# OpenDriveLab/ViDAR

Hardware: AMD Instinct MI355X
Metric: train samples/sec (6-cam->BEV step) (higher is better)
Workload: dtype f32

## Files before the change

### vidar_amd/csrc/dcn.hip

```cpp
#include <hip/hip_runtime.h>
#include <stdint.h>

#include "vidar_hip.h"
#include "vidar_common.h"
#include "det_scatter.h"

namespace {

struct PlaneTile { int plane, tile; bool ok; };
__device__ __forceinline__ PlaneTile xcd_plane_tile(int L, int T, int planes) {
  const int xcd = L & 7, j = L >> 3;
  const int pl = (j / T) * 8 + xcd;
  return PlaneTile{pl, j - (j / T) * T, pl < planes};
}
inline unsigned xcd_plane_grid(int T, int planes) { return 8u * (unsigned)T * (unsigned)((planes + 7) / 8); }

struct Conv { int C, H, W, Ho, Wo, kh, kw, stride, pad, dil; };

struct Bil {
  int h0, w0;
  float lh, lw;
  bool in, t, b, l, r;
};

__device__ __forceinline__ Bil bil(float h, float w, int H, int W) {
  Bil q;
  q.in = h > -1.f && w > -1.f && h < H && w < W;
  q.h0 = (int)floorf(h); q.w0 = (int)floorf(w);
  q.lh = h - q.h0; q.lw = w - q.w0;
  q.t = q.h0 >= 0; q.b = q.h0 + 1 <= H - 1; q.l = q.w0 >= 0; q.r = q.w0 + 1 <= W - 1;
  return q;
}

struct Pos { float h, w; };
__device__ __forceinline__ Pos tap_pos(const Conv& g, int py, int px, int t, float oh, float ow) {
  const int i = t / g.kw, j = t - i * g.kw;
  return Pos{py * g.stride - g.pad + i * g.dil + oh, px * g.stride - g.pad + j * g.dil + ow};
}

template <class F>
__device__ __forceinline__ void for_corners(const Bil& q, int W, F f) {
  const float hh = 1.f - q.lh, hw = 1.f - q.lw;
  const int tl = q.h0 * W + q.w0;
  if (q.t && q.l) f(tl, hh * hw);
  if (q.t && q.r) f(tl + 1, hh * q.lw);
  if (q.b && q.l) f(tl + W, q.lh * hw);
  if (q.b && q.r) f(tl + W + 1, q.lh * q.lw);
}

constexpr int kMaxTaps = 9;

typedef float pair_t __attribute__((ext_vector_type(2), aligned(4)));

template <bool PAIR>
__device__ __forceinline__ pair_t load_pair(const void* p) {
  if constexpr (PAIR) return *reinterpret_cast<const pair_t*>(p);
  else return pair_t{*reinterpret_cast<const float*>(p), 0.f};
}

struct PairMap {
  int top, bot;
  bool same, left;
  __device__ __forceinline__ float e0(float cl, float cr) const { return same ? cl : (left ? cr : 0.f); }
  __device__ __forceinline__ float e1(float cl, float cr) const { return same ? cr : (left ? 0.f : cl); }
};

__device__ __forceinline__ PairMap pair_map(const Bil& q, int H, int W) {
  const int c0 = min(max(q.w0, 0), max(W - 2, 0));
  const int r0 = min(max(q.h0, 0), H - 1), r1 = min(max(q.h0 + 1, 0), H - 1);
  return PairMap{r0 * W + c0, r1 * W + c0, q.w0 == c0, q.w0 < c0};
}

constexpr int kCP = 16;
struct TapFoot { unsigned top, bot; float wt0, wt1, wb0, wb1; };

__device__ __forceinline__ TapFoot tap_foot(Pos s, float m, const Conv& g) {
  const Bil q = bil(s.h, s.w, g.H, g.W);
  const PairMap pm = pair_map(q, g.H, g.W);
  const float wl = (q.l ? 1.f - q.lw : 0.f), wr = (q.r ? q.lw : 0.f);
  const float a0 = pm.e0(wl, wr), a1 = pm.e1(wl, wr);
  const float ht = (q.t ? 1.f - q.lh : 0.f) * m, hb = (q.b ? q.lh : 0.f) * m;
  TapFoot f;
  f.top = (unsigned)pm.top * 4u; f.bot = (unsigned)pm.bot * 4u;
  f.wt0 = q.in ? ht * a0 : 0.f; f.wt1 = q.in ? ht * a1 : 0.f;
  f.wb0 = q.in ? hb * a0 : 0.f; f.wb1 = q.in ? hb * a1 : 0.f;
  return f;
}

template <bool PAIR>
__device__ __forceinline__ void im2col_body(const float* __restrict__ x, const float* __restrict__ offset,
                                            const float* __restrict__ mask, float* __restrict__ cols, const Conv& g, int nimg) {
  const int P = g.Ho * g.Wo, K = g.kh * g.kw;
  const int cgroups = (g.C + kCP - 1) / kCP;
  const PlaneTile pt = xcd_plane_tile(blockIdx.x, (P + 255) / 256, cgroups * nimg);
  if (!pt.ok) return;
  const int p = pt.tile * 256 + threadIdx.x;
  if (p >= P) return;
  const int n = pt.plane / cgroups, c0 = (pt.plane - n * cgroups) * kCP, nc = min(kCP, g.C - c0);
  const int py = p / g.Wo, px = p % g.Wo;
  const size_t plane = (size_t)g.H * g.W, KP = (size_t)K * P;
  const char* im = reinterpret_cast<const char*>(x + ((size_t)n * g.C + c0) * plane);
  float* out = cols + ((size_t)n * g.C + c0) * KP + p;
  const float* off_n = offset + (size_t)n * 2 * K * P + p;
  const float* msk_n = mask + (size_t)n * K * P + p;
  float oh = off_n[0], ow = off_n[P], m = msk_n[0];
  for (int t = 0; t < K; ++t) {
    const TapFoot f = tap_foot(tap_pos(g, py, px, t, oh, ow), m, g);
    pair_t a[kCP], b[kCP];
#pragma unroll
    for (int c = 0; c < kCP; ++c) {
      const char* pl = im + (size_t)(c < nc ? c : 0) * plane * 4;
      a[c] = load_pair<PAIR>(pl + f.top);
      b[c] = load_pair<PAIR>(pl + f.bot);
    }
    if (t + 1 < K) {
      oh = off_n[(size_t)(2 * t + 2) * P]; ow = off_n[(size_t)(2 * t + 3) * P]; m = msk_n[(size_t)(t + 1) * P];
    }
#pragma unroll
    for (int c = 0; c < kCP; ++c)
      if (c < nc) {
        const float v = f.wt0 * a[c].x + f.wt1 * a[c].y + f.wb0 * b[c].x + f.wb1 * b[c].y;
        __builtin_nontemporal_store(v, out + (size_t)c * KP + (size_t)t * P);
      }
  }
}

__global__ __launch_bounds__(256) void dcn_im2col_pair_kernel(
    const float* __restrict__ x, const float* __restrict__ offset, const float* __restrict__ mask,
    float* __restrict__ cols, Conv g, int nimg) {
  im2col_body<true>(x, offset, mask, cols, g, nimg);
}
__global__ __launch_bounds__(256) void dcn_im2col_kernel(
    const float* __restrict__ x, const float* __restrict__ offset, const float* __restrict__ mask,
    float* __restrict__ cols, Conv g, int nimg) {
  im2col_body<false>(x, offset, mask, cols, g, nimg);
}

constexpr int kCG = 8;
template <class Acc>
__global__ __launch_bounds__(256) void dcn_col2im_kernel(const float* __restrict__ grad_cols, const float* __restrict__ offset,
                                                         const float* __restrict__ mask, float* __restrict__ grad_x, Conv g,
                                                         typename Acc::Param param) {
  Acc acc(grad_x, param);
  const int P = g.Ho * g.Wo, K = g.kh * g.kw;
  const int p = blockIdx.x * 256 + threadIdx.x;
  if constexpr (!Acc::kMeasureOnly) {
    if (p >= P) return;
  }
  const int n = blockIdx.z, c0 = blockIdx.y * kCG, nc = min(kCG, g.C - c0);
  const int py = p / g.Wo, px = p % g.Wo;
  const size_t plane = (size_t)g.H * g.W, KP = (size_t)K * P;
  float* gim = grad_x + ((size_t)n * g.C + c0) * plane;
  const float* gc = grad_cols + ((size_t)n * g.C + c0) * KP + p;
  for (int t = 0; t < K; ++t) {
    if constexpr (Acc::kMeasureOnly) {
      if (p >= P) break;
    }
    const size_t o = ((size_t)n * 2 * K + 2 * t) * P + p;
    const Pos s = tap_pos(g, py, px, t, offset[o], offset[o + P]);
    const Bil q = bil(s.h, s.w, g.H, g.W);
    if (!q.in) continue;
    const float m = mask[((size_t)n * K + t) * P + p];
    for (int c = 0; c < nc; ++c) {
      const float gv = gc[(size_t)c * KP + (size_t)t * P] * m;
      if (gv == 0.f) continue;
      for_corners(q, g.W, [&](int pix, float w) { acc.add(gim + (size_t)c * plane + pix, w * gv); });
    }
  }
  acc.flush();
}

struct Entry { int src; float w; };

template <bool FILL>
__global__ __launch_bounds__(256) void dcn_revmap_kernel(const float* __restrict__ offset,
                                                         const float* __restrict__ mask, int* __restrict__ cursor,
                                                         Entry* __restrict__ rec, Conv g) {
  const int P = g.Ho * g.Wo, K = g.kh * g.kw, HW = g.H * g.W;
  const int p = blockIdx.x * 256 + threadIdx.x;
  if (p >= P) return;
  const int t = blockIdx.y, n = blockIdx.z;
  const int py = p / g.Wo, px = p % g.Wo;
  const size_t o = ((size_t)n * 2 * K + 2 * t) * P + p;
  const Pos s = tap_pos(g, py, px, t, offset[o], offset[o + P]);
  const Bil q = bil(s.h, s.w, g.H, g.W);
  if (!q.in) return;
  const float m = FILL ? mask[((size_t)n * K + t) * P + p] : 0.f;
  int* cur = cursor + ((size_t)n * K + t) * HW;
  const int src = t * P + p;
  for_corners(q, g.W, [&](int pix, float w) {
    if (FILL) rec[atomicAdd(cur + pix, 1)] = Entry{src, w * m};
    else atomicAdd(cur + pix, 1);
  });
}

__global__ __launch_bounds__(1024) void dcn_revmap_scan_kernel(int* __restrict__ cursor, int* __restrict__ first,
                                                               int HW, int per_image) {
  __shared__ int s_part[1024];
  const int n = blockIdx.x;
  int* cnt = cursor + (size_t)n * HW;
  int* fst = first + (size_t)n * HW;
  const int per = (HW + 1023) / 1024;
  const int r0 = min(HW, (int)threadIdx.x * per), r1 = min(HW, r0 + per);
  int sum = 0;
  for (int i = r0; i < r1; ++i) sum += cnt[i];
  s_part[threadIdx.x] = sum;
  __syncthreads();
  for (int d = 1; d < 1024; d <<= 1) {
    const int a = (int)threadIdx.x >= d ? s_part[threadIdx.x - d] : 0;
    __syncthreads();
    s_part[threadIdx.x] += a;
    __syncthreads();
  }
  int run = n * per_image + s_part[threadIdx.x] - sum;
  for (int i = r0; i < r1; ++i) { const int c = cnt[i]; fst[i] = run; cnt[i] = run; run += c; }
}

constexpr int kGC = 16;
__global__ __launch_bounds__(256) void dcn_col2im_gather_kernel(const float* __restrict__ grad_cols,
                                                                const int* __restrict__ first,
                                                                const int* __restrict__ last,
                                                                const Entry* __restrict__ rec,
                                                                float* __restrict__ grad_x, Conv g) {
  const int P = g.Ho * g.Wo, K = g.kh * g.kw, HW = g.H * g.W;
  const int pix = blockIdx.x * 256 + threadIdx.x;
  if (pix >= HW) return;
  const int n = blockIdx.z, c0 = blockIdx.y * kGC;
  float acc[kGC];
#pragma unroll
  for (int c = 0; c < kGC; ++c) acc[c] = 0.f;
  const size_t KP = (size_t)K * P;
  const float* gc = grad_cols + ((size_t)n * g.C + c0) * KP;
  const int nc = min(kGC, g.C - c0);
  for (int t = 0; t < K; ++t) {
    const size_t bin = ((size_t)n * K + t) * HW + pix;
    const int e0 = first[bin], e1 = last[bin];
    if (nc == kGC) {
      int e = e0;
      for (; e + 1 < e1; e += 2) {
        const Entry r0 = rec[e], r1 = rec[e + 1];
        float v0[kGC], v1[kGC];
#pragma unroll
        for (int c = 0; c < kGC; ++c) { v0[c] = gc[(size_t)c * KP + r0.src]; v1[c] = gc[(size_t)c * KP + r1.src]; }
#pragma unroll
        for (int c = 0; c < kGC; ++c) acc[c] += r0.w * v0[c] + r1.w * v1[c];
      }
      if (e < e1) {
        const Entry r = rec[e];
#pragma unroll
        for (int c = 0; c < kGC; ++c) acc[c] += r.w * gc[(size_t)c * KP + r.src];
      }
    } else {
      for (int e = e0; e < e1; ++e) {
        const Entry r = rec[e];
        for (int c = 0; c < nc; ++c) acc[c] += r.w * gc[(size_t)c * KP + r.src];
      }
    }
  }
  for (int c = 0; c < nc; ++c) grad_x[((size_t)n * g.C + c0 + c) * HW + pix] = acc[c];
}

#ifndef VIDAR_DCN_GRY
#define VIDAR_DCN_GRY 2
#endif
#ifndef VIDAR_DCN_GLC
#define VIDAR_DCN_GLC 8
#endif
constexpr int kGRY = VIDAR_DCN_GRY;
constexpr int kGTH = 8 * kGRY, kGTW = 32;
#ifndef VIDAR_DCN_GHALO
#define VIDAR_DCN_GHALO 5
#endif
constexpr int kGHalo = VIDAR_DCN_GHALO;
constexpr int kGWH = kGTH + 2 * kGHalo + 2;
constexpr int kGWW = kGTW + 2 * kGHalo + 2;
constexpr int kGWP = (kGWW + 3) / 4 * 4;
constexpr int kGWS = kGWH * kGWP;
constexpr int kGLC = VIDAR_DCN_GLC;
constexpr int kGPos = (kGWS + 255) / 256;

__global__ __launch_bounds__(256) void dcn_col2im_gather_lds_kernel(
    const float* __restrict__ grad_cols, const int* __restrict__ first, const int* __restrict__ last,
    const Entry* __restrict__ rec, float* __restrict__ grad_x, Conv g, int tiles_x, int tiles_y, int nimg, float inv_wo) {
  __shared__ __attribute__((aligned(16))) float s_gc[kGLC * kGWS];
  constexpr int K = 9;
  const int P = g.Ho * g.Wo, HW = g.H * g.W;
  const int cgroups = (g.C + kGLC - 1) / kGLC;
  const PlaneTile pt = xcd_plane_tile(blockIdx.x, tiles_x * tiles_y, cgroups * nimg);
  if (!pt.ok) return;
  const int tile = pt.tile, tyi = tile / tiles_x, txi = tile - tyi * tiles_x;
  const int n = pt.plane / cgroups, c0 = (pt.plane - n * cgroups) * kGLC, nc = min(kGLC, g.C - c0);
  const int ry = threadIdx.x / kGTW, rx = threadIdx.x % kGTW;
  const int dx = txi * kGTW + rx;
  const size_t KP = (size_t)K * P;
  const float* gc = grad_cols + ((size_t)n * g.C + c0) * KP;
  float acc[kGRY][kGLC];
#pragma unroll
  for (int k = 0; k < kGRY; ++k)
#pragma unroll
    for (int c = 0; c < kGLC; ++c) acc[k][c] = 0.f;
  for (int t = 0; t < K; ++t) {
    const int i = t / 3, j = t - i * 3;
    const int wy0 = tyi * kGTH + g.pad - i - kGHalo - 1, wx0 = txi * kGTW + g.pad - j - kGHalo - 1;
    const float* gct = gc + (size_t)t * P;
    __syncthreads();
    {
      const int wave = __builtin_amdgcn_readfirstlane((int)threadIdx.x >> 6);
#pragma unroll
      for (int k = 0; k < kGPos; ++k) {
        const int e = threadIdx.x + k * 256;
        const int r = e / kGWP, cc = e - r * kGWP;
        const int sy = wy0 + r, sx = wx0 + cc;
        const bool ok = e < kGWS && sy >= 0 && sy < g.Ho && sx >= 0 && sx < g.Wo && cc < kGWW;
        const int off = ok ? sy * g.Wo + sx : 0;
        if (ok) {
#pragma unroll
          for (int c = 0; c < kGLC; ++c)
            __builtin_amdgcn_global_load_lds((const __attribute__((address_space(1))) void*)(gct + (size_t)(c < nc ? c : 0) * KP + off),
                                             (__attribute__((address_space(3))) void*)(s_gc + c * kGWS + k * 256 + wave * 64), 4, 0, 0);
        }
      }
    }
    __syncthreads();
    if (dx >= g.W) continue;
#pragma unroll
    for (int k = 0; k < kGRY; ++k) {
      const int dy = tyi * kGTH + ry + 8 * k;
      if (dy >= g.H) continue;
      const size_t bin = ((size_t)n * K + t) * HW + dy * g.W + dx;
      const int e1 = last[bin];
      int e = first[bin];
      Entry nxt = e < e1 ? rec[e] : Entry{0, 0.f};
      while (e < e1) {
        const Entry r = nxt;
        ++e;
        if (e < e1) nxt = rec[e];
        const int p = r.src - t * P;
        const int py = (int)((p + 0.5f) * inv_wo), px = p - py * g.Wo;
        const int ly = py - wy0, lx = px - wx0;
        if (ly >= 0 && ly < kGWH && lx >= 0 && lx < kGWW) {
          const float* q = s_gc + ly * kGWP + lx;
#pragma unroll
          for (int c = 0; c < kGLC; ++c) acc[k][c] += r.w * q[c * kGWS];
        } else {
          for (int c = 0; c < nc; ++c) acc[k][c] += r.w * gct[(size_t)c * KP + p];
        }
      }
    }
  }
  if (dx < g.W) {
#pragma unroll
    for (int k = 0; k < kGRY; ++k) {
      const int dy = tyi * kGTH + ry + 8 * k;
      if (dy < g.H)
        for (int c = 0; c < nc; ++c) grad_x[((size_t)n * g.C + c0 + c) * HW + dy * g.W + dx] = acc[k][c];
    }
  }
}

int g_dcn_variant = 1;

template <bool PAIR>
__device__ __forceinline__ void col2im_coord_body(const float* __restrict__ grad_cols, const float* __restrict__ x,
                                                  const float* __restrict__ offset, const float* __restrict__ mask,
                                                  float* __restrict__ grad_offset, float* __restrict__ grad_mask,
                                                  const Conv& g) {
  const int P = g.Ho * g.Wo, K = g.kh * g.kw;
  const int p = blockIdx.x * 256 + threadIdx.x;
  if (p >= P) return;
  const int t = blockIdx.y, n = blockIdx.z;
  const int py = p / g.Wo, px = p % g.Wo;
  const size_t o = ((size_t)n * 2 * K + 2 * t) * P + p;
  const Pos s = tap_pos(g, py, px, t, offset[o], offset[o + P]);
  const float m = mask[((size_t)n * K + t) * P + p];
  const Bil q = bil(s.h, s.w, g.H, g.W);
  float gh = 0.f, gw = 0.f, gm = 0.f;
  if (q.in) {
    const float hh = 1.f - q.lh, hw = 1.f - q.lw;
    const PairMap pm = pair_map(q, g.H, g.W);
    const float tl = (q.t && q.l) ? 1.f : 0.f, tr = (q.t && q.r) ? 1.f : 0.f;
    const float bl = (q.b && q.l) ? 1.f : 0.f, br = (q.b && q.r) ? 1.f : 0.f;
    const float m_t0 = pm.e0(hh * hw * tl, hh * q.lw * tr), m_t1 = pm.e1(hh * hw * tl, hh * q.lw * tr);
    const float m_b0 = pm.e0(q.lh * hw * bl, q.lh * q.lw * br), m_b1 = pm.e1(q.lh * hw * bl, q.lh * q.lw * br);
    const float h_t0 = pm.e0(-hw * tl, -q.lw * tr), h_t1 = pm.e1(-hw * tl, -q.lw * tr);
    const float h_b0 = pm.e0(hw * bl, q.lw * br), h_b1 = pm.e1(hw * bl, q.lw * br);
    const float w_t0 = pm.e0(-hh * tl, hh * tr), w_t1 = pm.e1(-hh * tl, hh * tr);
    const float w_b0 = pm.e0(-q.lh * bl, q.lh * br), w_b1 = pm.e1(-q.lh * bl, q.lh * br);
    int c = 0;
    constexpr int kCB = 8;
    const unsigned top_b = (unsigned)pm.top * 4u, bot_b = (unsigned)pm.bot * 4u, p_b = (unsigned)p * 4u;
    const size_t plane_b = (size_t)g.H * g.W * 4, col_b = (size_t)K * P * 4;
    for (; c + kCB <= g.C; c += kCB) {
      const char* im0 = reinterpret_cast<const char*>(x) + ((size_t)n * g.C + c) * plane_b;
      const char* gc0 = reinterpret_cast<const char*>(grad_cols) + (((size_t)n * g.C + c) * K + t) * (size_t)P * 4;
      pair_t a[kCB], b[kCB];
      float gc[kCB];
#pragma unroll
      for (int u = 0; u < kCB; ++u) {
        gc[u] = *reinterpret_cast<const float*>(gc0 + u * col_b + p_b);
        a[u] = load_pair<PAIR>(im0 + u * plane_b + top_b);
        b[u] = load_pair<PAIR>(im0 + u * plane_b + bot_b);
      }
      __builtin_amdgcn_sched_barrier(0);
#pragma unroll
      for (int u = 0; u < kCB; ++u) {
        gm += gc[u] * (m_t0 * a[u].x + m_t1 * a[u].y + m_b0 * b[u].x + m_b1 * b[u].y);
        gh += gc[u] * (h_t0 * a[u].x + h_t1 * a[u].y + h_b0 * b[u].x + h_b1 * b[u].y);
        gw += gc[u] * (w_t0 * a[u].x + w_t1 * a[u].y + w_b0 * b[u].x + w_b1 * b[u].y);
      }
    }
    for (; c < g.C; ++c) {
      const float* im = x + ((size_t)n * g.C + c) * g.H * g.W;
      const float gc = grad_cols[(((size_t)n * g.C + c) * K + t) * P + p];
      const pair_t a = load_pair<PAIR>(im + pm.top), b = load_pair<PAIR>(im + pm.bot);
      gm += gc * (m_t0 * a.x + m_t1 * a.y + m_b0 * b.x + m_b1 * b.y);
      gh += gc * (h_t0 * a.x + h_t1 * a.y + h_b0 * b.x + h_b1 * b.y);
      gw += gc * (w_t0 * a.x + w_t1 * a.y + w_b0 * b.x + w_b1 * b.y);
    }
  }
  grad_offset[o] = gh * m;
  grad_offset[o + P] = gw * m;
  grad_mask[((size_t)n * K + t) * P + p] = gm;
}

__global__ __launch_bounds__(256) void dcn_col2im_coord_kernel(
    const float* __restrict__ grad_cols, const float* __restrict__ x, const float* __restrict__ offset,
    const float* __restrict__ mask, float* __restrict__ grad_offset, float* __restrict__ grad_mask, Conv g) {
  col2im_coord_body<true>(grad_cols, x, offset, mask, grad_offset, grad_mask, g);
}
__global__ __launch_bounds__(256) void dcn_col2im_coord_1col_kernel(
    const float* __restrict__ grad_cols, const float* __restrict__ x, const float* __restrict__ offset,
    const float* __restrict__ mask, float* __restrict__ grad_offset, float* __restrict__ grad_mask, Conv g) {
  col2im_coord_body<false>(grad_cols, x, offset, mask, grad_offset, grad_mask, g);
}

inline bool dcn_bad(int N, const Conv& g) {
  return N < 0 || g.C <= 0 || g.H <= 0 || g.W <= 0 || g.Ho <= 0 || g.Wo <= 0 || g.kh <= 0 ||
         g.kw <= 0 || g.stride <= 0 || g.dil <= 0 || g.pad < 0;
}

}

extern "C" {

int vidar_dcn_set_variant(int variant) {
  const int prev = g_dcn_variant;
  if (variant >= 0 && variant <= 1) g_dcn_variant = variant;
  return prev;
}

int vidar_dcn_im2col_f32(const float* x, const float* offset, const float* mask, float* cols, int N,
                         int C, int H, int W, int Ho, int Wo, int kh, int kw, int stride, int pad,
                         int dil, void* stream) {
  VIDAR_ENTER();
  Conv g{C, H, W, Ho, Wo, kh, kw, stride, pad, dil};
  if (dcn_bad(N, g)) return VIDAR_ERR_BAD_ARG;
  if (N == 0) return 0;
  if (kh * kw > kMaxTaps) return VIDAR_ERR_BAD_ARG;
  hipLaunchKernelGGL(W >= 2 ? dcn_im2col_pair_kernel : dcn_im2col_kernel,
                     dim3(xcd_plane_grid((Ho * Wo + 255) / 256, ((C + kCP - 1) / kCP) * N)), dim3(256), 0, (hipStream_t)stream,
                     x, offset, mask, cols, g, N);
  return vidar_last_error();
}

size_t vidar_dcn_col2im_workspace_bytes(int N, int H, int W, int Ho, int Wo, int kh, int kw) {
  if (N <= 0 || H <= 0 || W <= 0 || Ho <= 0 || Wo <= 0 || kh <= 0 || kw <= 0) return 0;
  const size_t hw = (size_t)N * kh * kw * H * W, ent = (size_t)N * kh * kw * Ho * Wo * 4;
  if (ent >= (1ull << 31)) return 0;
  return sizeof(int) * 2 * hw + sizeof(Entry) * ent;
}

int vidar_dcn_col2im_det_workspace_bytes(int N, int C, int H, int W, int64_t* bytes) {
  if (N < 0 || C < 0 || H < 0 || W < 0 || !bytes) return VIDAR_ERR_BAD_ARG;
  *bytes = (int64_t)det_workspace_bytes((size_t)N * C * H * W);
  return 0;
}

int vidar_dcn_col2im_f32(const float* grad_cols, const float* x, const float* offset,
                         const float* mask, float* grad_x, float* grad_offset, float* grad_mask,
                         int N, int C, int H, int W, int Ho, int Wo, int kh, int kw, int stride,
                         int pad, int dil, void* workspace, size_t workspace_bytes, void* stream) {
  VIDAR_ENTER();
  Conv g{C, H, W, Ho, Wo, kh, kw, stride, pad, dil};
  if (dcn_bad(N, g)) return VIDAR_ERR_BAD_ARG;
  hipStream_t s = (hipStream_t)stream;
  if (N == 0) return 0;
  if (kh * kw > kMaxTaps) return VIDAR_ERR_BAD_ARG;
  const int P = Ho * Wo, K = kh * kw, HW = H * W;
  if (det_mode()) {
    const dim3 grid((P + 255) / 256, (C + kCG - 1) / kCG, N);
    const int rc = det_scatter(
        grad_x, nullptr, (size_t)N * C * HW, 0, (uint64_t)N * C * K * P * 4, false, workspace, workspace_bytes, s,
        [&](auto tag, auto param, auto) {
          hipLaunchKernelGGL(dcn_col2im_kernel<decltype(tag)>, grid, dim3(256), 0, s, grad_cols, offset, mask, grad_x, g,
                             param);
        });
    if (rc != 0) return rc;
  } else if (workspace) {
    const size_t need = vidar_dcn_col2im_workspace_bytes(N, H, W, Ho, Wo, kh, kw);
    if (need == 0 || workspace_bytes < need) return VIDAR_ERR_BAD_ARG;
    int* cursor = (int*)workspace;
    int* first = cursor + (size_t)N * K * HW;
    Entry* rec = (Entry*)(first + (size_t)N * K * HW);
    hipError_t e = hipMemsetAsync(cursor, 0, sizeof(int) * (size_t)N * K * HW, s);
    if (e != hipSuccess) return (int)e;
    const dim3 rgrid((P + 255) / 256, K, N);
    hipLaunchKernelGGL(dcn_revmap_kernel<false>, rgrid, dim3(256), 0, s, offset, mask, cursor, rec, g);
    hipLaunchKernelGGL(dcn_revmap_scan_kernel, dim3(N * K), dim3(1024), 0, s, cursor, first, HW, P * 4);
    hipLaunchKernelGGL(dcn_revmap_kernel<true>, rgrid, dim3(256), 0, s, offset, mask, cursor, rec, g);
    if ((g_dcn_variant & 1) && kh == 3 && kw == 3 && stride == 1 && dil == 1 && Ho == H && Wo == W) {
      const int tiles_x = (W + kGTW - 1) / kGTW, tiles_y = (H + kGTH - 1) / kGTH;
      hipLaunchKernelGGL(dcn_col2im_gather_lds_kernel, dim3(xcd_plane_grid(tiles_x * tiles_y, ((C + kGLC - 1) / kGLC) * N)), dim3(256), 0,
                         s, grad_cols, first, cursor, rec, grad_x, g, tiles_x, tiles_y, N, 1.0f / (float)Wo);
    } else {
      hipLaunchKernelGGL(dcn_col2im_gather_kernel, dim3((HW + 255) / 256, (C + kGC - 1) / kGC, N), dim3(256), 0, s,
                         grad_cols, first, cursor, rec, grad_x, g);
    }
  } else {
    hipError_t e = hipMemsetAsync(grad_x, 0, sizeof(float) * (size_t)N * C * H * W, s);
    if (e != hipSuccess) return (int)e;
    hipLaunchKernelGGL(dcn_col2im_kernel<det::AccAtomic>, dim3((P + 255) / 256, (C + kCG - 1) / kCG, N), dim3(256), 0, s, grad_cols,
                       offset, mask, grad_x, g, det::AccAtomic::Param{});
  }
  hipLaunchKernelGGL(W >= 2 ? dcn_col2im_coord_kernel : dcn_col2im_coord_1col_kernel, dim3((P + 255) / 256, K, N), dim3(256), 0,
                     s, grad_cols, x, offset, mask, grad_offset, grad_mask, g);
  return vidar_last_error();
}

}
```

Baseline: 2.949.

## Split DCN coord-gradient channel loop across wavefront slices with LDS reduction

The DCN offset/mask gradient kernel can now split the channel reduction across S wavefronts per block (64 pixels per block), with each slice handling a contiguous channel range and the partial sums reduced through shared memory. When the grid is small (fewer than 1024 base blocks), four slices are used to raise parallelism and the number of loads in flight. The new variant bit is enabled by default. It adds a block barrier and LDS traffic, and changes the order of the floating-point summation.

```diff
diff --git a/vidar_amd/csrc/dcn.hip b/vidar_amd/csrc/dcn.hip
--- a/vidar_amd/csrc/dcn.hip
+++ b/vidar_amd/csrc/dcn.hip
@@ -358,80 +358,119 @@
   }
 }
 
-int g_dcn_variant = 1;
-
-template <bool PAIR>
+int g_dcn_variant = 3;
+
+#ifndef VIDAR_DCN_COORD_S
+#define VIDAR_DCN_COORD_S 0
+#endif
+template <bool PAIR, int S>
 __device__ __forceinline__ void col2im_coord_body(const float* __restrict__ grad_cols, const float* __restrict__ x,
                                                   const float* __restrict__ offset, const float* __restrict__ mask,
                                                   float* __restrict__ grad_offset, float* __restrict__ grad_mask,
                                                   const Conv& g) {
   const int P = g.Ho * g.Wo, K = g.kh * g.kw;
-  const int p = blockIdx.x * 256 + threadIdx.x;
-  if (p >= P) return;
+  constexpr int kCB = 8;
+  const int lane = S == 1 ? (int)threadIdx.x : (int)threadIdx.x & 63;
+  const int slice = S == 1 ? 0 : __builtin_amdgcn_readfirstlane((int)threadIdx.x >> 6);
+  const int p = blockIdx.x * (S == 1 ? 256 : 64) + lane;
+  const bool live = p < P;
+  if constexpr (S == 1) {
+    if (!live) return;
+  }
+  const int per = (((g.C + S - 1) / S + kCB - 1) / kCB) * kCB;
+  const int cb = min(slice * per, g.C), ce = min(cb + per, g.C);
   const int t = blockIdx.y, n = blockIdx.z;
   const int py = p / g.Wo, px = p % g.Wo;
   const size_t o = ((size_t)n * 2 * K + 2 * t) * P + p;
-  const Pos s = tap_pos(g, py, px, t, offset[o], offset[o + P]);
-  const float m = mask[((size_t)n * K + t) * P + p];
-  const Bil q = bil(s.h, s.w, g.H, g.W);
-  float gh = 0.f, gw = 0.f, gm = 0.f;
-  if (q.in) {
-    const float hh = 1.f - q.lh, hw = 1.f - q.lw;
-    const PairMap pm = pair_map(q, g.H, g.W);
-    const float tl = (q.t && q.l) ? 1.f : 0.f, tr = (q.t && q.r) ? 1.f : 0.f;
-    const float bl = (q.b && q.l) ? 1.f : 0.f, br = (q.b && q.r) ? 1.f : 0.f;
-    const float m_t0 = pm.e0(hh * hw * tl, hh * q.lw * tr), m_t1 = pm.e1(hh * hw * tl, hh * q.lw * tr);
-    const float m_b0 = pm.e0(q.lh * hw * bl, q.lh * q.lw * br), m_b1 = pm.e1(q.lh * hw * bl, q.lh * q.lw * br);
-    const float h_t0 = pm.e0(-hw * tl, -q.lw * tr), h_t1 = pm.e1(-hw * tl, -q.lw * tr);
-    const float h_b0 = pm.e0(hw * bl, q.lw * br), h_b1 = pm.e1(hw * bl, q.lw * br);
-    const float w_t0 = pm.e0(-hh * tl, hh * tr), w_t1 = pm.e1(-hh * tl, hh * tr);
-    const float w_b0 = pm.e0(-q.lh * bl, q.lh * br), w_b1 = pm.e1(-q.lh * bl, q.lh * br);
-    int c = 0;
-    constexpr int kCB = 8;
-    const unsigned top_b = (unsigned)pm.top * 4u, bot_b = (unsigned)pm.bot * 4u, p_b = (unsigned)p * 4u;
-    const size_t plane_b = (size_t)g.H * g.W * 4, col_b = (size_t)K * P * 4;
-    for (; c + kCB <= g.C; c += kCB) {
-      const char* im0 = reinterpret_cast<const char*>(x) + ((size_t)n * g.C + c) * plane_b;
-      const char* gc0 = reinterpret_cast<const char*>(grad_cols) + (((size_t)n * g.C + c) * K + t) * (size_t)P * 4;
-      pair_t a[kCB], b[kCB];
-      float gc[kCB];
-#pragma unroll
-      for (int u = 0; u < kCB; ++u) {
-        gc[u] = *reinterpret_cast<const float*>(gc0 + u * col_b + p_b);
-        a[u] = load_pair<PAIR>(im0 + u * plane_b + top_b);
-        b[u] = load_pair<PAIR>(im0 + u * plane_b + bot_b);
-      }
-      __builtin_amdgcn_sched_barrier(0);
-#pragma unroll
-      for (int u = 0; u < kCB; ++u) {
-        gm += gc[u] * (m_t0 * a[u].x + m_t1 * a[u].y + m_b0 * b[u].x + m_b1 * b[u].y);
-        gh += gc[u] * (h_t0 * a[u].x + h_t1 * a[u].y + h_b0 * b[u].x + h_b1 * b[u].y);
-        gw += gc[u] * (w_t0 * a[u].x + w_t1 * a[u].y + w_b0 * b[u].x + w_b1 * b[u].y);
-      }
-    }
-    for (; c < g.C; ++c) {
-      const float* im = x + ((size_t)n * g.C + c) * g.H * g.W;
-      const float gc = grad_cols[(((size_t)n * g.C + c) * K + t) * P + p];
-      const pair_t a = load_pair<PAIR>(im + pm.top), b = load_pair<PAIR>(im + pm.bot);
-      gm += gc * (m_t0 * a.x + m_t1 * a.y + m_b0 * b.x + m_b1 * b.y);
-      gh += gc * (h_t0 * a.x + h_t1 * a.y + h_b0 * b.x + h_b1 * b.y);
-      gw += gc * (w_t0 * a.x + w_t1 * a.y + w_b0 * b.x + w_b1 * b.y);
-    }
+  float gh = 0.f, gw = 0.f, gm = 0.f, m = 0.f;
+  if (live) {
+    const Pos s = tap_pos(g, py, px, t, offset[o], offset[o + P]);
+    m = mask[((size_t)n * K + t) * P + p];
+    const Bil q = bil(s.h, s.w, g.H, g.W);
+    if (q.in) {
+      const float hh = 1.f - q.lh, hw = 1.f - q.lw;
+      const PairMap pm = pair_map(q, g.H, g.W);
+      const float tl = (q.t && q.l) ? 1.f : 0.f, tr = (q.t && q.r) ? 1.f : 0.f;
+      const float bl = (q.b && q.l) ? 1.f : 0.f, br = (q.b && q.r) ? 1.f : 0.f;
+      const float m_t0 = pm.e0(hh * hw * tl, hh * q.lw * tr), m_t1 = pm.e1(hh * hw * tl, hh * q.lw * tr);
+      const float m_b0 = pm.e0(q.lh * hw * bl, q.lh * q.lw * br), m_b1 = pm.e1(q.lh * hw * bl, q.lh * q.lw * br);
+      const float h_t0 = pm.e0(-hw * tl, -q.lw * tr), h_t1 = pm.e1(-hw * tl, -q.lw * tr);
+      const float h_b0 = pm.e0(hw * bl, q.lw * br), h_b1 = pm.e1(hw * bl, q.lw * br);
+      const float w_t0 = pm.e0(-hh * tl, hh * tr), w_t1 = pm.e1(-hh * tl, hh * tr);
+      const float w_b0 = pm.e0(-q.lh * bl, q.lh * br), w_b1 = pm.e1(-q.lh * bl, q.lh * br);
+      int c = cb;
+      const unsigned top_b = (unsigned)pm.top * 4u, bot_b = (unsigned)pm.bot * 4u, p_b = (unsigned)p * 4u;
+      const size_t plane_b = (size_t)g.H * g.W * 4, col_b = (size_t)K * P * 4;
+      for (; c + kCB <= ce; c += kCB) {
+        const char* im0 = reinterpret_cast<const char*>(x) + ((size_t)n * g.C + c) * plane_b;
+        const char* gc0 = reinterpret_cast<const char*>(grad_cols) + (((size_t)n * g.C + c) * K + t) * (size_t)P * 4;
+        pair_t a[kCB], b[kCB];
+        float gc[kCB];
+#pragma unroll
+        for (int u = 0; u < kCB; ++u) {
+          gc[u] = *reinterpret_cast<const float*>(gc0 + u * col_b + p_b);
+          a[u] = load_pair<PAIR>(im0 + u * plane_b + top_b);
+          b[u] = load_pair<PAIR>(im0 + u * plane_b + bot_b);
+        }
+        __builtin_amdgcn_sched_barrier(0);
+#pragma unroll
+        for (int u = 0; u < kCB; ++u) {
+          gm += gc[u] * (m_t0 * a[u].x + m_t1 * a[u].y + m_b0 * b[u].x + m_b1 * b[u].y);
+          gh += gc[u] * (h_t0 * a[u].x + h_t1 * a[u].y + h_b0 * b[u].x + h_b1 * b[u].y);
+          gw += gc[u] * (w_t0 * a[u].x + w_t1 * a[u].y + w_b0 * b[u].x + w_b1 * b[u].y);
+        }
+      }
+      for (; c < ce; ++c) {
+        const float* im = x + ((size_t)n * g.C + c) * g.H * g.W;
+        const float gc = grad_cols[(((size_t)n * g.C + c) * K + t) * P + p];
+        const pair_t a = load_pair<PAIR>(im + pm.top), b = load_pair<PAIR>(im + pm.bot);
+        gm += gc * (m_t0 * a.x + m_t1 * a.y + m_b0 * b.x + m_b1 * b.y);
+        gh += gc * (h_t0 * a.x + h_t1 * a.y + h_b0 * b.x + h_b1 * b.y);
+        gw += gc * (w_t0 * a.x + w_t1 * a.y + w_b0 * b.x + w_b1 * b.y);
+      }
+    }
+  }
+  if constexpr (S > 1) {
+    __shared__ float s_part[S - 1][3][64];
+    if (slice > 0) {
+      s_part[slice - 1][0][lane] = gm; s_part[slice - 1][1][lane] = gh; s_part[slice - 1][2][lane] = gw;
+    }
+    __syncthreads();
+    if (slice > 0 || !live) return;
+#pragma unroll
+    for (int k = 0; k < S - 1; ++k) { gm += s_part[k][0][lane]; gh += s_part[k][1][lane]; gw += s_part[k][2][lane]; }
   }
   grad_offset[o] = gh * m;
   grad_offset[o + P] = gw * m;
   grad_mask[((size_t)n * K + t) * P + p] = gm;
 }
 
-__global__ __launch_bounds__(256) void dcn_col2im_coord_kernel(
+template <bool PAIR, int S>
+__global__ __launch_bounds__(S == 1 ? 256 : 64 * S) void dcn_col2im_coord_kernel(
     const float* __restrict__ grad_cols, const float* __restrict__ x, const float* __restrict__ offset,
     const float* __restrict__ mask, float* __restrict__ grad_offset, float* __restrict__ grad_mask, Conv g) {
-  col2im_coord_body<true>(grad_cols, x, offset, mask, grad_offset, grad_mask, g);
-}
-__global__ __launch_bounds__(256) void dcn_col2im_coord_1col_kernel(
-    const float* __restrict__ grad_cols, const float* __restrict__ x, const float* __restrict__ offset,
-    const float* __restrict__ mask, float* __restrict__ grad_offset, float* __restrict__ grad_mask, Conv g) {
-  col2im_coord_body<false>(grad_cols, x, offset, mask, grad_offset, grad_mask, g);
+  col2im_coord_body<PAIR, S>(grad_cols, x, offset, mask, grad_offset, grad_mask, g);
+}
+
+inline int coord_slices(int P, int K, int N) {
+  if (VIDAR_DCN_COORD_S) return VIDAR_DCN_COORD_S;
+  return (long long)((P + 255) / 256) * K * N < 256 * 4 ? 4 : 1;
+}
+
+template <bool PAIR>
+void launch_coord(int S, hipStream_t s, const float* grad_cols, const float* x, const float* offset, const float* mask,
+                  float* grad_offset, float* grad_mask, const Conv& g, int N) {
+  const int P = g.Ho * g.Wo, K = g.kh * g.kw;
+  const dim3 grid((P + (S == 1 ? 255 : 63)) / (S == 1 ? 256 : 64), K, N), block(S == 1 ? 256 : 64 * S);
+  auto go = [&](auto kernel) {
+    hipLaunchKernelGGL(kernel, grid, block, 0, s, grad_cols, x, offset, mask, grad_offset, grad_mask, g);
+  };
+  switch (S) {
+    case 2: go(dcn_col2im_coord_kernel<PAIR, 2>); break;
+    case 4: go(dcn_col2im_coord_kernel<PAIR, 4>); break;
+    case 8: go(dcn_col2im_coord_kernel<PAIR, 8>); break;
+    default: go(dcn_col2im_coord_kernel<PAIR, 1>);
+  }
 }
 
 inline bool dcn_bad(int N, const Conv& g) {
@@ -445,7 +484,7 @@
 
 int vidar_dcn_set_variant(int variant) {
   const int prev = g_dcn_variant;
-  if (variant >= 0 && variant <= 1) g_dcn_variant = variant;
+  if (variant >= 0 && variant <= 3) g_dcn_variant = variant;
   return prev;
 }
 
@@ -522,8 +561,9 @@
     hipLaunchKernelGGL(dcn_col2im_kernel<det::AccAtomic>, dim3((P + 255) / 256, (C + kCG - 1) / kCG, N), dim3(256), 0, s, grad_cols,
                        offset, mask, grad_x, g, det::AccAtomic::Param{});
   }
-  hipLaunchKernelGGL(W >= 2 ? dcn_col2im_coord_kernel : dcn_col2im_coord_1col_kernel, dim3((P + 255) / 256, K, N), dim3(256), 0,
-                     s, grad_cols, x, offset, mask, grad_offset, grad_mask, g);
+  const int S = (g_dcn_variant & 2) || det_mode() ? coord_slices(P, K, N) : 1;
+  if (W >= 2) launch_coord<true>(S, s, grad_cols, x, offset, mask, grad_offset, grad_mask, g, N);
+  else launch_coord<false>(S, s, grad_cols, x, offset, mask, grad_offset, grad_mask, g, N);
   return vidar_last_error();
 }
 
```

Result: no change. 2.948 (median of 2 runs) (-0.0%).
